# koide3/glim

Measured on NVIDIA H100. Metric: VGICP linearize throughput, higher is better.
Workload: dtype f32

## Files before the change

### glim_b200/csrc/gb_kernels_vgicp.cu

```cuda
#include "gb_internal.cuh"
#include "gb_vgicp_math.cuh"

#include "gb_sweep_steps.cuh"

namespace {

constexpr int kSubMax = 512;
constexpr int kLookupUnroll3 = 5;
constexpr int kRound3 = 32 * kLookupUnroll3 * ((kSubMax - 31) / (32 * kLookupUnroll3));
static_assert(kRound3 + 31 <= kSubMax, "a round's hits and the up to 31 carried from the previous round fit the queue");

template <int MODE, bool PEER, bool SV>
__global__ void __launch_bounds__(kThreads, 2) k_vgicp_sweep3(
  const FactorDesc* __restrict__ descs, const double* __restrict__ poses, const double* __restrict__ poses_eval,
  const int2* __restrict__ items, int num_items,
  unsigned long long* __restrict__ item_ctr, unsigned long long ctr_base,
  double* __restrict__ accum, int acc_slots, unsigned* __restrict__ done, double* __restrict__ out, float* __restrict__ slab, const PeerPush* __restrict__ peer) {
  __shared__ __align__(16) uint2 s_q[kWarps][kSubMax];
  const int lane = threadIdx.x & 31, warp = threadIdx.x >> 5;
  const unsigned lt_mask = (1u << lane) - 1u;
  uint2* __restrict__ q = s_q[warp];
  auto desc_of = [&](int f) { return descs[f]; };

  const int total_warps = gridDim.x * kWarps;
  const bool dynamic = num_items > total_warps;
  int item = blockIdx.x * kWarps + warp;
  if (item >= num_items) return;
  int2 it = __ldg(&items[item]);
  int pend_f = -1, pend_last = 0, pend_tiles = 0;
  auto pend_count = [&] { return pend_tiles; };

  while (true) {
    int next_item = 0x7fffffff;
    if (dynamic && lane == 0) next_item = (int)(atomicAdd(item_ctr, 1ull) - ctr_base) + total_warps;
    const int f = it.x;
    const FactorDesc D = descs[f];
    const PoseF P = pose_from_colmajor(poses + (size_t)f * 16);
    PoseF Pe = P;
    if (MODE == GB_MODE_ERROR) Pe = pose_from_colmajor(poses_eval + (size_t)f * 16);
    const int item_end = min(it.y + D.chunk, D.n);
    bool published = pend_f < 0;
    float acc[32];
#pragma unroll
    for (int k = 0; k < 32; k++) acc[k] = 0.f;

    int nq = 0;
    for (int wb = it.y; wb < item_end; wb += kRound3) {
      const int we = min(wb + kRound3, item_end);
      for (int i0 = wb; i0 < we; i0 += 32 * kLookupUnroll3) {
        Probe p[kLookupUnroll3];
#pragma unroll
        for (int u = 0; u < kLookupUnroll3; u++) {
          const float4 a0 = __ldg(&D.p0[min(i0 + u * 32 + lane, we - 1)]);
          probe_issue(D, P, a0.x, a0.y, a0.z, p[u]);
        }
        if (!published) {
          published = true;
          __syncwarp();
          if (lane == 0) pend_last = ticket_last(done, pend_f, pend_count);
        }
        int v[kLookupUnroll3];
        probe_resolve(D, p, v);
#pragma unroll
        for (int u = 0; u < kLookupUnroll3; u++) probe_compact(v[u], i0 + u * 32 + lane, we, q, nq, lt_mask);
      }
      __syncwarp();
      const int nacc = we == item_end ? nq : (nq & ~31);
      accumulate_queue<MODE, SV>(acc, D, P, Pe, q, nacc, lane);
      __syncwarp();
      nq -= nacc;
      if (nacc > 0 && lane < nq) q[lane] = q[nacc + lane];
      __syncwarp();
    }
    if (!published) {
      __syncwarp();
      if (lane == 0) pend_last = ticket_last(done, pend_f, pend_count);
    }

    reduce_item<MODE>(acc, accum, f, acc_slots, item, lane);
    if (pend_f >= 0 && __shfl_sync(0xffffffffu, pend_last, 0)) {
      fence_acquire();
      retire_factor<MODE, PEER>(pend_f, desc_of(pend_f), poses, poses_eval, accum, acc_slots, out, slab, peer, q);
      __syncwarp();
    }
    pend_f = f; pend_tiles = D.num_tiles; pend_last = 0;
    item = __shfl_sync(0xffffffffu, next_item, 0);
    if (item >= num_items) break;
    it = __ldg(&items[item]);
  }
  __syncwarp();
  if (lane == 0) pend_last = ticket_last(done, pend_f, pend_count);
  if (__shfl_sync(0xffffffffu, pend_last, 0)) {
    fence_acquire();
    retire_factor<MODE, PEER>(pend_f, desc_of(pend_f), poses, poses_eval, accum, acc_slots, out, slab, peer, q);
  }
}

constexpr int kLookupUnroll5 = 4;
constexpr int kDescCache = 40;
struct CtaCache {
  FactorDesc desc[kDescCache];
  PoseF pose[kDescCache];
  PoseF pose_eval[kDescCache];
};

template <int MODE, bool PEER>
__global__ void __launch_bounds__(kThreads, 2) k_vgicp_sweep5(
  const FactorDesc* __restrict__ descs, int num_factors, const double* __restrict__ poses, const double* __restrict__ poses_eval,
  const int2* __restrict__ items, int num_items,
  unsigned long long* __restrict__ item_ctr, unsigned long long ctr_base,
  double* __restrict__ accum, int acc_slots, unsigned* __restrict__ done, double* __restrict__ out, float* __restrict__ slab, const PeerPush* __restrict__ peer) {
  __shared__ __align__(16) uint2 s_q[kWarps][kSubMax];
  __shared__ CtaCache cache_s;
  CtaCache* const cache = &cache_s;
  constexpr int U = kLookupUnroll5;
  constexpr int kGroupsPerRound = kSubMax / (32 * U);
  const int lane = threadIdx.x & 31, warp = threadIdx.x >> 5;
  const unsigned lt_mask = (1u << lane) - 1u;
  uint2* __restrict__ q = s_q[warp];

  const bool cached = num_factors <= kDescCache;
  if (cached) {
    for (int f = threadIdx.x; f < num_factors; f += kThreads) {
      cache->desc[f] = descs[f];
      cache->pose[f] = pose_from_colmajor(poses + (size_t)f * 16);
      if (MODE == GB_MODE_ERROR) cache->pose_eval[f] = pose_from_colmajor(poses_eval + (size_t)f * 16);
    }
    __syncthreads();
  }
  auto desc_of = [&](int f) -> FactorDesc { FactorDesc d; if (cached) d = cache->desc[f]; else d = descs[f]; return d; };

  const int total_warps = gridDim.x * kWarps;
  const bool dynamic = num_items > total_warps;
  int item = blockIdx.x * kWarps + warp;
  if (item >= num_items) return;
  int nxt = 0x7fffffff;
  if (dynamic) {
    if (lane == 0) nxt = (int)(atomicAdd(item_ctr, 1ull) - ctr_base) + total_warps;
    nxt = __shfl_sync(0xffffffffu, nxt, 0);
  }
  int2 it = __ldg(&items[item]);
  int pend_f = -1, pend_last = 0;
  auto pend_count = [&] { return desc_of(pend_f).num_tiles; };

  while (true) {
    int nxt2 = 0x7fffffff;
    if (dynamic && lane == 0) nxt2 = (int)(atomicAdd(item_ctr, 1ull) - ctr_base) + total_warps;
    int2 it_next = make_int2(0, 0);
    if (nxt < num_items) it_next = __ldg(&items[nxt]);
    const int f = it.x;
    const FactorDesc D = desc_of(f);
    PoseF P;
    if (cached) P = cache->pose[f]; else P = pose_from_colmajor(poses + (size_t)f * 16);
    PoseF Pe = P;
    if (MODE == GB_MODE_ERROR) { if (cached) Pe = cache->pose_eval[f]; else Pe = pose_from_colmajor(poses_eval + (size_t)f * 16); }

    const int limit = D.n;
    const int row_stride = D.num_tiles * 32;
    const int first = it.y * 32;
    int ngroups = 0;
    if (first < limit) {
      const int rows = (limit - first + row_stride - 1) / row_stride;
      ngroups = (rows + U - 1) / U;
    }

    float acc[32];
#pragma unroll
    for (int k = 0; k < 32; k++) acc[k] = 0.f;
    bool published = (pend_f < 0);

    for (int g0 = 0; g0 < ngroups; g0 += kGroupsPerRound) {
      const int g1 = min(g0 + kGroupsPerRound, ngroups);
      int nq = 0;
      float ax[U], ay[U], az[U];
#pragma unroll
      for (int u = 0; u < U; u++) {
        const int i = first + (g0 * U + u) * row_stride + lane;
        const float4 a0 = __ldg(&D.p0[i < limit ? i : 0]);
        ax[u] = a0.x; ay[u] = a0.y; az[u] = a0.z;
      }
      for (int g = g0; g < g1; g++) {
        Probe p[U];
#pragma unroll
        for (int u = 0; u < U; u++) probe_issue(D, P, ax[u], ay[u], az[u], p[u]);
        if (!published) {
          published = true;
          __syncwarp();
          if (lane == 0) pend_last = ticket_last(done, pend_f, pend_count);
        }
        int v[U];
        probe_resolve(D, p, v);
#pragma unroll
        for (int u = 0; u < U; u++) probe_compact(v[u], first + (g * U + u) * row_stride + lane, limit, q, nq, lt_mask);
        if (g + 1 < g1) {
#pragma unroll
          for (int u = 0; u < U; u++) {
            const int i = first + ((g + 1) * U + u) * row_stride + lane;
            const float4 a0 = __ldg(&D.p0[i < limit ? i : 0]);
            ax[u] = a0.x; ay[u] = a0.y; az[u] = a0.z;
          }
        }
      }
      __syncwarp();
      accumulate_queue<MODE, true>(acc, D, P, Pe, q, nq, lane);
      __syncwarp();
    }
    if (!published) {
      __syncwarp();
      if (lane == 0) pend_last = ticket_last(done, pend_f, pend_count);
    }

    reduce_item<MODE>(acc, accum, f, acc_slots, item, lane);
    if (pend_f >= 0 && __shfl_sync(0xffffffffu, pend_last, 0)) {
      fence_acquire();
      retire_factor<MODE, PEER>(pend_f, desc_of(pend_f), poses, poses_eval, accum, acc_slots, out, slab, peer, q);
      __syncwarp();
    }
    pend_f = f;
    pend_last = 0;
    item = nxt;
    it = it_next;
    nxt = __shfl_sync(0xffffffffu, nxt2, 0);
    if (item >= num_items) break;
  }
  __syncwarp();
  if (lane == 0) pend_last = ticket_last(done, pend_f, pend_count);
  if (__shfl_sync(0xffffffffu, pend_last, 0)) {
    fence_acquire();
    retire_factor<MODE, PEER>(pend_f, desc_of(pend_f), poses, poses_eval, accum, acc_slots, out, slab, peer, q);
  }
}

__global__ void __launch_bounds__(256) k_overlap(int num_targets, const FactorDesc* __restrict__ descs, const double* __restrict__ poses, int n, int* __restrict__ count) {
  extern __shared__ float s_poses[];
  for (int k = threadIdx.x; k < num_targets * 12; k += blockDim.x) {
    const int t = k / 12, e = k % 12;
    const int r = e < 9 ? e / 3 : e - 9, c = e < 9 ? e % 3 : 3;
    s_poses[k] = (float)poses[(size_t)t * 16 + c * 4 + r];
  }
  __syncthreads();
  int local = 0;
  const FactorDesc D0 = descs[0];
  for (int i = blockIdx.x * blockDim.x + threadIdx.x; i < n; i += gridDim.x * blockDim.x) {
    const float4 a0 = __ldg(&D0.p0[i]);
    for (int t = 0; t < num_targets; t++) {
      const PoseF P = load_pose(s_poses + 12 * t);
      float qx, qy, qz;
      transform(P, a0.x, a0.y, a0.z, qx, qy, qz);
      const float sum = (qx + qy) + qz;
      if (!(sum == sum)) continue;
      const float inv_res = descs[t].inv_res;
      const int v = gb_lookup(descs[t].buckets, descs[t].mask, descs[t].max_scan, gb_coord(qx, inv_res), gb_coord(qy, inv_res), gb_coord(qz, inv_res));
      if (v >= 0) { local++; break; }
    }
  }
#pragma unroll
  for (int o = 16; o >= 1; o >>= 1) local += __shfl_xor_sync(0xffffffffu, local, o);
  if ((threadIdx.x & 31) == 0 && local) atomicAdd(count, local);
}

}

template <int MODE, bool PEER>
static gb_status launch5(gb_sweep* s, const double* poses_eval, float* slab, const PeerPush* pp) {
  return gb_launch(s->ctx, "k_vgicp_sweep5", k_vgicp_sweep5<MODE, PEER>, s->grid, kThreads, 0, s->d_descs, (int)s->F, s->d_poses, poses_eval, s->d_tiles, s->num_tiles, s->d_tile_ctr,
                   s->ctr_base, s->d_accum, s->acc_slots, s->d_done, s->d_out, slab, pp);
}

template <int MODE, bool PEER, bool SV>
static gb_status launch3(gb_sweep* s, const double* poses_eval, float* slab, const PeerPush* pp) {
  return gb_launch(s->ctx, "k_vgicp_sweep3", k_vgicp_sweep3<MODE, PEER, SV>, s->grid, kThreads, 0, s->d_descs, s->d_poses, poses_eval, s->d_tiles, s->num_tiles, s->d_tile_ctr,
                   s->ctr_base, s->d_accum, s->acc_slots, s->d_done, s->d_out, slab, pp);
}

gb_status gb_launch_sweep(gb_sweep* s, int mode) {
  if (s->num_tiles == 0) return GB_OK;
  if (s->gicp) return gb_launch_gicp_sweep(s, mode);
  const bool peer = (mode == GB_MODE_LINEARIZE) && s->peer != nullptr;
  const PeerPush* pp = peer ? s->d_peer_tables + s->peer->parity : nullptr;
  float* slab = mode == GB_MODE_LINEARIZE ? s->d_slab : nullptr;
  const double* pe = mode == GB_MODE_ERROR ? s->d_poses_eval : nullptr;
  gb_status st;
  if (s->kernel_version == 3) {
    if (s->any_sv) {
      if (mode == GB_MODE_LINEARIZE) st = peer ? launch3<GB_MODE_LINEARIZE, true, true>(s, pe, slab, pp) : launch3<GB_MODE_LINEARIZE, false, true>(s, pe, slab, pp);
      else st = launch3<GB_MODE_ERROR, false, true>(s, pe, slab, pp);
    } else {
      if (mode == GB_MODE_LINEARIZE) st = peer ? launch3<GB_MODE_LINEARIZE, true, false>(s, pe, slab, pp) : launch3<GB_MODE_LINEARIZE, false, false>(s, pe, slab, pp);
      else st = launch3<GB_MODE_ERROR, false, false>(s, pe, slab, pp);
    }
  } else {
    if (mode == GB_MODE_LINEARIZE) st = peer ? launch5<GB_MODE_LINEARIZE, true>(s, pe, slab, pp) : launch5<GB_MODE_LINEARIZE, false>(s, pe, slab, pp);
    else st = launch5<GB_MODE_ERROR, false>(s, pe, slab, pp);
  }
  GB_CHECK(st);
  const unsigned long long warps = (unsigned long long)s->grid * kWarps;
  if ((unsigned long long)s->num_tiles > warps) s->ctr_base += (s->kernel_version == 3 ? 0ull : warps) + (unsigned long long)s->num_tiles;
  return GB_OK;
}

gb_status gb_launch_overlap(gb_ctx* ctx, int num_targets, const FactorDesc* d_descs, const double* d_poses, int n, int* d_count) {
  if (n <= 0 || num_targets <= 0) return GB_OK;
  const int grid = min((n + 255) / 256, ctx->num_sms * 8);
  return gb_launch(ctx, "k_overlap", k_overlap, grid, 256, (size_t)num_targets * 12 * sizeof(float), num_targets, d_descs, d_poses, n, d_count);
}
```

Measured before the change: 108,700.

## Park sweep3 accumulators in shared memory between rounds and widen lookup unroll

The per-item accumulators no longer stay live in registers across the lookup phase. They are spilled to a per-warp shared-memory slot after each accumulate round and reloaded before the next one. The freed registers let the lookup unroll grow to 8 or 7 probes per lane, depending on mode, to give more memory-level parallelism. To fit the parked accumulators in shared memory, the per-warp queue shrinks from 512 to 304 entries. That means shorter rounds and more frequent accumulate passes, plus extra shared-memory traffic for parking.

```diff
diff --git a/glim_b200/csrc/gb_kernels_vgicp.cu b/glim_b200/csrc/gb_kernels_vgicp.cu
--- a/glim_b200/csrc/gb_kernels_vgicp.cu
+++ b/glim_b200/csrc/gb_kernels_vgicp.cu
@@ -5,10 +5,16 @@
 
 namespace {
 
-constexpr int kSubMax = 512;
-constexpr int kLookupUnroll3 = 5;
-constexpr int kRound3 = 32 * kLookupUnroll3 * ((kSubMax - 31) / (32 * kLookupUnroll3));
-static_assert(kRound3 + 31 <= kSubMax, "a round's hits and the up to 31 carried from the previous round fit the queue");
+constexpr int kQueue3 = 304;
+struct Sweep3Warp {
+  uint2 q[kQueue3];
+  float acc[29][32];
+};
+static_assert(sizeof(Sweep3Warp) * kWarps <= 48 * 1024, "static shared memory");
+template <int MODE, bool SV> constexpr int kLookupUnroll3 = SV ? 5 : MODE == GB_MODE_LINEARIZE ? 8 : 7;
+template <int MODE, bool SV> constexpr int kRound3 = 32 * kLookupUnroll3<MODE, SV> * ((kQueue3 - 31) / (32 * kLookupUnroll3<MODE, SV>));
+static_assert(kRound3<GB_MODE_LINEARIZE, false> > 0 && kRound3<GB_MODE_ERROR, false> > 0 && kRound3<GB_MODE_LINEARIZE, true> > 0,
+              "a round's hits and the up to 31 carried from the previous round fit the queue");
 
 template <int MODE, bool PEER, bool SV>
 __global__ void __launch_bounds__(kThreads, 2) k_vgicp_sweep3(
@@ -16,11 +22,13 @@
   const int2* __restrict__ items, int num_items,
   unsigned long long* __restrict__ item_ctr, unsigned long long ctr_base,
   double* __restrict__ accum, int acc_slots, unsigned* __restrict__ done, double* __restrict__ out, float* __restrict__ slab, const PeerPush* __restrict__ peer) {
-  __shared__ __align__(16) uint2 s_q[kWarps][kSubMax];
+  __shared__ __align__(16) Sweep3Warp s_w[kWarps];
   const int lane = threadIdx.x & 31, warp = threadIdx.x >> 5;
   const unsigned lt_mask = (1u << lane) - 1u;
-  uint2* __restrict__ q = s_q[warp];
+  uint2* __restrict__ q = s_w[warp].q;
+  float (*__restrict__ parked)[32] = s_w[warp].acc;
   auto desc_of = [&](int f) { return descs[f]; };
+  constexpr int U = kLookupUnroll3<MODE, SV>, kRound = kRound3<MODE, SV>;
 
   const int total_warps = gridDim.x * kWarps;
   const bool dynamic = num_items > total_warps;
@@ -40,17 +48,19 @@
     if (MODE == GB_MODE_ERROR) Pe = pose_from_colmajor(poses_eval + (size_t)f * 16);
     const int item_end = min(it.y + D.chunk, D.n);
     bool published = pend_f < 0;
-    float acc[32];
-#pragma unroll
-    for (int k = 0; k < 32; k++) acc[k] = 0.f;
+    bool held = false;
+    auto unpark = [&](float (&acc)[32]) {
+#pragma unroll
+      for (int k = 0; k < 32; k++) acc[k] = held && k < 29 && (MODE == GB_MODE_LINEARIZE || k >= 27) ? parked[k][lane] : 0.f;
+    };
 
     int nq = 0;
-    for (int wb = it.y; wb < item_end; wb += kRound3) {
-      const int we = min(wb + kRound3, item_end);
-      for (int i0 = wb; i0 < we; i0 += 32 * kLookupUnroll3) {
-        Probe p[kLookupUnroll3];
-#pragma unroll
-        for (int u = 0; u < kLookupUnroll3; u++) {
+    for (int wb = it.y; wb < item_end; wb += kRound) {
+      const int we = min(wb + kRound, item_end);
+      for (int i0 = wb; i0 < we; i0 += 32 * U) {
+        Probe p[U];
+#pragma unroll
+        for (int u = 0; u < U; u++) {
           const float4 a0 = __ldg(&D.p0[min(i0 + u * 32 + lane, we - 1)]);
           probe_issue(D, P, a0.x, a0.y, a0.z, p[u]);
         }
@@ -59,14 +69,22 @@
           __syncwarp();
           if (lane == 0) pend_last = ticket_last(done, pend_f, pend_count);
         }
-        int v[kLookupUnroll3];
+        int v[U];
         probe_resolve(D, p, v);
 #pragma unroll
-        for (int u = 0; u < kLookupUnroll3; u++) probe_compact(v[u], i0 + u * 32 + lane, we, q, nq, lt_mask);
+        for (int u = 0; u < U; u++) probe_compact(v[u], i0 + u * 32 + lane, we, q, nq, lt_mask);
       }
       __syncwarp();
       const int nacc = we == item_end ? nq : (nq & ~31);
-      accumulate_queue<MODE, SV>(acc, D, P, Pe, q, nacc, lane);
+      if (nacc > 0) {
+        float acc[32];
+        unpark(acc);
+        accumulate_queue<MODE, SV>(acc, D, P, Pe, q, nacc, lane);
+#pragma unroll
+        for (int k = 0; k < 29; k++)
+          if (MODE == GB_MODE_LINEARIZE || k >= 27) parked[k][lane] = acc[k];
+        held = true;
+      }
       __syncwarp();
       nq -= nacc;
       if (nacc > 0 && lane < nq) q[lane] = q[nacc + lane];
@@ -77,6 +95,8 @@
       if (lane == 0) pend_last = ticket_last(done, pend_f, pend_count);
     }
 
+    float acc[32];
+    unpark(acc);
     reduce_item<MODE>(acc, accum, f, acc_slots, item, lane);
     if (pend_f >= 0 && __shfl_sync(0xffffffffu, pend_last, 0)) {
       fence_acquire();
@@ -96,6 +116,7 @@
   }
 }
 
+constexpr int kSubMax = 512;
 constexpr int kLookupUnroll5 = 4;
 constexpr int kDescCache = 40;
 struct CtaCache {
```

Result: faster. 113,900, median of 6 (+4.8%).
